# aiforvision/OCTA-autosegmentation

Hardware: AMD Instinct MI355X
Metric: synthetic OCTA samples/sec (graph + 304x304 image + 1216x1216 label triples) (higher is better)
Workload: dtype f64

## Files before the change

### include/octa_hip.h

```cpp
#ifndef OCTA_HIP_H
#define OCTA_HIP_H

#include <stddef.h>
#include <stdint.h>

#ifdef __cplusplus
extern "C" {
#endif

typedef struct octa_ctx octa_ctx;


int octa_abi_version(void);

const char *octa_last_error(void);

int octa_ctx_create(int device, octa_ctx **out);
void octa_ctx_destroy(octa_ctx *ctx);

size_t octa_ctx_scratch_bytes(const octa_ctx *ctx);

int octa_rasterize_2d(octa_ctx *ctx, int B, const double *d_edges, const int64_t *h_edge_off,
                      const uint8_t *d_keep, int no_pixels_x, int no_pixels_y, int mip_axis,
                      double min_radius, double max_radius, uint8_t *d_out, void *stream);
// ... 284 lines not shown
int octa_sim_geometry(int num_cus, int *h_out4);

int octa_sim_is_large(const octa_sim *sim);

int octa_sim_fields(octa_sim *sim, int sample, double *h_oxy, int64_t cap_oxy, int64_t *n_oxy, double *h_co2,
                    int64_t cap_co2, int64_t *n_co2);

int octa_sim_kat_kd_order(octa_ctx *ctx, const double *h_pts, int64_t n, const uint8_t *h_need, int32_t *h_indices);

int octa_sim_kat_kd_order_signflag(octa_ctx *ctx, const double *h_pts, int64_t n, const uint8_t *h_need, int32_t need_bits, int32_t *h_indices);

int octa_sim_kat_sample(octa_ctx *ctx, const double *h_cand, int64_t n_cand, const double *h_npos, const double *h_nrad, int64_t n_art,
                        double *h_oxy, int64_t n_oxy, int64_t cap_oxy, double eps_n, double eps_k, double eps_s, const double *h_cst8,
                        int64_t *h_n_out);

#ifdef __cplusplus
}
#endif
#endif
```

### octa_autosegmentation_amd/_native.py

```python
import contextlib
import ctypes
import os
import random as _random
import threading

import numpy as np

HERE = os.path.dirname(os.path.abspath(__file__))
LIB_PATH = os.environ.get("OCTA_HIP_LIB") or os.path.join(HERE, "liboctahip.so")

_lib = None
_ctxs = {}
_lock = threading.Lock()

c_void_p, c_int, c_double, c_size_t = ctypes.c_void_p, ctypes.c_int, ctypes.c_double, ctypes.c_size_t


def _struct(name, ints, ptrs):
    fields = [("struct_size", ctypes.c_uint32)] + [(k, c_int) for k in ints.split()] + [("slope", ctypes.c_float)] + [(k, c_void_p) for k in ptrs.split()]
    return type(name, (ctypes.Structure,), {"_fields_": fields})


Conv3x3Args = _struct("Conv3x3Args", "N H W Cin Cout stride in_dilation tap_mask out_scale out_off_y out_off_x C1 CY1 nslot",
                      "d_x d_x2 d_w d_y d_y2 d_scale1 d_shift1 d_scale2 d_shift2 d_stat_partials d_stat_slots d_residual")
# ... 113 lines not shown
    "octa_headn_nhwc_bwd": (c_int, [c_void_p, c_void_p, c_void_p, c_void_p, c_int, ctypes.c_int64, c_int, c_int, c_void_p, c_void_p, c_void_p, c_void_p]),
    "octa_conv3x3_c1_fwd": (c_int, [c_void_p, c_void_p, c_void_p, c_void_p, c_int, c_int, c_int, c_int, c_void_p, c_int, c_void_p]),
    "octa_fft2_c2c_f64_workspace_bytes": (c_size_t, [c_int, c_int, c_int]),
    "octa_fft2_c2c_f64": (c_int, [c_void_p, c_void_p, c_int, c_int, c_int, c_int, c_void_p, c_void_p]),
    "octa_oof_workspace_bytes": (c_size_t, [c_int, c_int, c_int]),
    "octa_oof_2d": (c_int, [c_void_p, c_void_p, c_int, c_int, c_int, c_void_p, c_void_p]),
    "octa_oof_2d_response": (c_int, [c_void_p, c_void_p, c_int, c_int, c_int, c_void_p, c_void_p]),
    "octa_frangi_workspace_bytes": (c_size_t, [c_int, c_int, c_int, c_int]),
    "octa_frangi_2d": (c_int, [c_void_p, c_void_p, c_int, c_int, c_int, c_int, c_void_p, c_void_p, ctypes.c_float, c_double, c_double, c_int, c_void_p, c_void_p]),
    "octa_frangi_hessian": (c_int, [c_void_p, c_void_p, c_void_p, c_void_p, c_int, c_int, c_int, c_int, c_void_p, ctypes.c_float, c_int, c_void_p, c_void_p]),
    "octa_frangi_eigenvalues": (c_int, [c_void_p, c_void_p, c_void_p, c_void_p, c_int, c_int, c_int, c_int, c_void_p, ctypes.c_float, c_int, c_void_p, c_void_p]),
    "octa_sim_kat_kd_order": (c_int, [c_void_p, c_void_p, ctypes.c_int64, c_void_p, c_void_p]),
    "octa_sim_kat_kd_order_signflag": (c_int, [c_void_p, c_void_p, ctypes.c_int64, c_void_p, ctypes.c_int32, c_void_p]),
    "octa_sim_kat_sample": (c_int, [c_void_p, c_void_p, ctypes.c_int64, c_void_p, c_void_p, ctypes.c_int64, c_void_p, ctypes.c_int64, ctypes.c_int64,
                                    c_double, c_double, c_double, c_void_p, c_void_p]),
}


class OctaHipError(RuntimeError):
    pass


def lib():
    global _lib
    if _lib is None:
        with _lock:
            if _lib is None:
                if not os.path.exists(LIB_PATH):
                    raise OctaHipError(
                        f"{LIB_PATH} is missing: build it with `python -m octa_autosegmentation_amd.build` "
# ... 113 lines not shown
```

### octa_autosegmentation_amd/csrc/sim.hip

```cpp

#include <chrono>
#include <vector>

#include "common.h"
#include "sim_host.h"
#include <thread>
#include <atomic>
#include <cstdlib>
#include <cstring>

using namespace OCTA_SIMK;

#if OCTA_SIM_LARGE
#define OCTA_SIM_T octa_simL_impl
#define OCTA_SIM_FN(name) octa_simL_##name
#else
#define OCTA_SIM_T octa_simS_impl
#define OCTA_SIM_FN(name) octa_simS_##name
#endif
#define octa_sim_create OCTA_SIM_FN(create)
#define octa_sim_destroy OCTA_SIM_FN(destroy)
#define octa_sim_run OCTA_SIM_FN(run)
#define octa_sim_run_states OCTA_SIM_FN(run_states)
#define octa_sim_np_state OCTA_SIM_FN(np_state)
#define octa_sim_edge_offsets OCTA_SIM_FN(edge_offsets)
#define octa_sim_export_edges OCTA_SIM_FN(export_edges)
#define octa_sim_export_edges_device OCTA_SIM_FN(export_edges_device)
#define octa_sim_trace OCTA_SIM_FN(trace)
#define octa_sim_stats OCTA_SIM_FN(stats)
#define octa_sim_kd_paths OCTA_SIM_FN(kd_paths)
#define octa_sim_assign_paths OCTA_SIM_FN(assign_paths)
#define octa_sim_fields OCTA_SIM_FN(fields)
#define octa_sim_service_stats OCTA_SIM_FN(service_stats)
#define octa_sim_geometry OCTA_SIM_FN(geometry)
#define octa_sim_spans OCTA_SIM_FN(spans)
#define octa_sim_timing OCTA_SIM_FN(timing)
#define octa_sim_kat_kd_order OCTA_SIM_FN(kat_kd_order)
#define octa_sim_kat_kd_order_signflag OCTA_SIM_FN(kat_kd_order_signflag)
#define octa_sim_kat_sample OCTA_SIM_FN(kat_sample)
struct OCTA_SIM_T;
extern "C" void octa_sim_destroy(OCTA_SIM_T *S);
extern "C" long long octa_sim_next_ticket(void);
extern "C" int *octa_sim_launch_flag(int device);

namespace {

constexpr int SIM_THREADS = SIM_THREADS_PER_WG;
constexpr int SIM_WG_PER_CU = 2;
#if OCTA_SIM_LARGE
constexpr size_t SIM_LDS = 2048;
#else
constexpr size_t SIM_LDS = SIM_LDS_BYTES;
static_assert((size_t)KD_MAILBOX_OFF + KD_MAILBOX_BYTES <= (size_t)SIM_USER_BYTES && SIM_WG_PER_CU * SIM_LDS <= 160 * 1024, "LDS budget");
#endif
// ... 1306 lines not shown
    hipLaunchKernelGGL(sim_kat_kd_kernel, dim3(1), dim3(SIM_THREADS), SIM_LDS, 0, d_pts, (int)n, d_need, d_idx, d_idx + n, d_xy, zlo, zhi, flag_in_sign, need_bits);
    OCTA_HIP_CHECK(hipGetLastError());
    std::vector<idx_t> h(n);
    OCTA_HIP_CHECK(hipMemcpy(h.data(), d_idx, sizeof(idx_t) * n, hipMemcpyDeviceToHost));
    for (int64_t i = 0; i < n; i++) h_indices[i] = (int32_t)h[i];
    (void)hipFree(d_pts); (void)hipFree(d_idx); (void)hipFree(d_xy); if (d_need) (void)hipFree(d_need);
    return 0;
}

__global__ void __launch_bounds__(SIM_THREADS)
sim_kat_sample_kernel(SimArrays A, SimConst C, IterParams P) {
    extern __shared__ __attribute__((aligned(16))) unsigned char smem[];
    Blk b = {(int)threadIdx.x, (int)blockDim.x, smem};
    phase_sample(b, A, C, P, 0);
}
}

extern "C" int octa_sim_kat_sample(octa_ctx *ctx, const double *h_cand, int64_t n_cand, const double *h_npos, const double *h_nrad, int64_t n_art,
                                   double *h_oxy, int64_t n_oxy, int64_t cap_oxy, double eps_n, double eps_k, double eps_s, const double *h_cst8,
                                   int64_t *h_n_out) {
    if (!ctx || !h_cst8 || !h_n_out || n_cand < 0 || n_cand > NCANDCAP || n_art < 0 || n_art > NCAP || n_oxy < 0 || n_oxy > OCAP || cap_oxy < n_oxy ||
        (n_cand && !h_cand) || (n_art && (!h_npos || !h_nrad)) || (cap_oxy && !h_oxy)) {
        octa::set_error("octa_sim_kat_sample: bad arguments");
        return -2;
    }
    OCTA_HIP_CHECK(hipSetDevice(ctx->device));
    SimConst C;
    memset(&C, 0, sizeof(C));
    C.ps = h_cst8[0]; C.sx = h_cst8[1]; C.sy = h_cst8[2]; C.sz = h_cst8[3]; C.gs = h_cst8[4]; C.fc0 = h_cst8[5]; C.fc1 = h_cst8[6];
    SampleScalars sc;
// ... 67 lines not shown
```

### octa_autosegmentation_amd/csrc/sim_api.cpp

```cpp
#include <cstdlib>
#include <cstring>
#include <new>

#include "common.h"

extern "C" {
struct octa_simS_impl;
struct octa_simL_impl;
#define OCTA_DECL(SFX, T)                                                                                                                       \
    int octa_sim##SFX##_create(octa_ctx *, const octa_sim_config *, int, T **);                                                                 \
    void octa_sim##SFX##_destroy(T *);                                                                                                          \
    int octa_sim##SFX##_run(T *, const uint32_t *, const uint64_t *, octa_bif_fn, void *, void *);                                              \
    int octa_sim##SFX##_run_states(T *, const double *, const double *, const uint32_t *, const uint32_t *, octa_bif_fn, void *, void *);       \
    int octa_sim##SFX##_np_state(T *, int, uint32_t *);                                                                                         \
    int octa_sim##SFX##_edge_offsets(T *, int64_t *, int64_t *);                                                                                \
    int octa_sim##SFX##_export_edges(T *, double *);                                                                                            \
    int octa_sim##SFX##_export_edges_device(T *, double *, void *);                                                                             \
    int octa_sim##SFX##_trace(T *, int32_t *);                                                                                                  \
    int octa_sim##SFX##_stats(T *, int64_t *);                                                                                                  \
    int octa_sim##SFX##_kd_paths(T *, int64_t *);                                                                                               \
    int octa_sim##SFX##_assign_paths(T *, int64_t *);                                                                                           \
    int octa_sim##SFX##_spans(T *, int64_t *);                                                                                                  \
    int octa_sim##SFX##_timing(T *, double *);                                                                                                  \
    int octa_sim##SFX##_service_stats(T *, double *);                                                                                           \
    int octa_sim##SFX##_geometry(int, int *);                                                                                                   \
    int octa_sim##SFX##_fields(T *, int, double *, int64_t, int64_t *, double *, int64_t, int64_t *);
OCTA_DECL(S, octa_simS_impl)
OCTA_DECL(L, octa_simL_impl)
#undef OCTA_DECL
int octa_simS_kat_kd_order(octa_ctx *, const double *, int64_t, const uint8_t *, int32_t *);
int octa_simS_kat_kd_order_signflag(octa_ctx *, const double *, int64_t, const uint8_t *, int32_t, int32_t *);
int octa_simS_kat_sample(octa_ctx *, const double *, int64_t, const double *, const double *, int64_t, double *, int64_t, int64_t, double, double, double,
                         const double *, int64_t *);
}

#include <atomic>
#include <mutex>
static std::atomic<long long> g_sim_launches{0};
extern "C" long long octa_sim_next_ticket(void) { return g_sim_launches.fetch_add(1, std::memory_order_acq_rel) + 1; }
extern "C" long long octa_sim_launch_count(void) { return g_sim_launches.load(std::memory_order_acquire); }
extern "C" int *octa_sim_launch_flag(int device) {
    static std::mutex m;
    static int *flags[64] = {};
    if (device < 0 || device >= 64) return nullptr;
    std::lock_guard<std::mutex> g(m);
    if (!flags[device]) {
        int prev = 0;
        if (hipGetDevice(&prev) != hipSuccess || hipSetDevice(device) != hipSuccess) return nullptr;
// ... 62 lines not shown
extern "C" int octa_sim_kd_paths(octa_sim *sim, int64_t *t) { NEED(sim, "octa_sim_kd_paths") return FWD(octa_simS_kd_paths(sim->s, t), octa_simL_kd_paths(sim->l, t)); }
extern "C" int octa_sim_assign_paths(octa_sim *sim, int64_t *t) { NEED(sim, "octa_sim_assign_paths") return FWD(octa_simS_assign_paths(sim->s, t), octa_simL_assign_paths(sim->l, t)); }
extern "C" int octa_sim_spans(octa_sim *sim, int64_t *t) { NEED(sim, "octa_sim_spans") return FWD(octa_simS_spans(sim->s, t), octa_simL_spans(sim->l, t)); }
extern "C" int octa_sim_timing(octa_sim *sim, double *t) { NEED(sim, "octa_sim_timing") return FWD(octa_simS_timing(sim->s, t), octa_simL_timing(sim->l, t)); }
extern "C" int octa_sim_service_stats(octa_sim *sim, double *t) { NEED(sim, "octa_sim_service_stats") return FWD(octa_simS_service_stats(sim->s, t), octa_simL_service_stats(sim->l, t)); }
extern "C" int octa_sim_fields(octa_sim *sim, int k, double *o, int64_t co, int64_t *no, double *c, int64_t cc, int64_t *nc) {
    NEED(sim, "octa_sim_fields") return FWD(octa_simS_fields(sim->s, k, o, co, no, c, cc, nc), octa_simL_fields(sim->l, k, o, co, no, c, cc, nc));
}
extern "C" int octa_sim_geometry(int num_cus, int *h_out4) { return octa_simS_geometry(num_cus, h_out4); }
extern "C" int octa_sim_kat_kd_order(octa_ctx *ctx, const double *p, int64_t n, const uint8_t *need, int32_t *o) { return octa_simS_kat_kd_order(ctx, p, n, need, o); }
extern "C" int octa_sim_kat_kd_order_signflag(octa_ctx *ctx, const double *p, int64_t n, const uint8_t *need, int32_t bits, int32_t *o) { return octa_simS_kat_kd_order_signflag(ctx, p, n, need, bits, o); }
extern "C" int octa_sim_kat_sample(octa_ctx *ctx, const double *cand, int64_t n_cand, const double *npos, const double *nrad, int64_t n_art, double *oxy,
                                   int64_t n_oxy, int64_t cap_oxy, double eps_n, double eps_k, double eps_s, const double *cst8, int64_t *n_out) {
    return octa_simS_kat_sample(ctx, cand, n_cand, npos, nrad, n_art, oxy, n_oxy, cap_oxy, eps_n, eps_k, eps_s, cst8, n_out);
}
extern "C" int octa_sim_is_large(const octa_sim *sim) { return sim && sim->large ? 1 : 0; }
```

### octa_autosegmentation_amd/csrc/sim_core.h

```cpp
#pragma once
#include <cmath>
#include <cstdint>
#include <cstring>
#include <algorithm>
#include "gpow.h"
#include "glibc_trig.h"

#ifndef OCTA_SIM_LARGE
#define OCTA_SIM_LARGE 0
#endif
#if OCTA_SIM_LARGE
#define OCTA_SIMK octa_simk_large
#else
#define OCTA_SIMK octa_simk
#endif
namespace OCTA_SIMK {

#if OCTA_SIM_LARGE
typedef unsigned int idx_t;
typedef unsigned long long kdw_t;
constexpr int IDX_BITS = 18;
constexpr int GROUP_BITS = 17;
constexpr int NCAP = 1 << 17;
constexpr int OCAP = 1 << 18;
// ... 282 lines not shown
    for (int i0 = s0; i0 < s1; i0 += 64) {
        const bool keep = i0 + lane < s1 && pred(i0 + lane);
        const unsigned long long m = __ballot(keep);
        if (keep) emit(i0 + lane, at + (int)__popcll(m & ((1ull << lane) - 1ull)));
        at += (int)__popcll(m);
    }
    return tot;
#else
    (void)b;
    int at = 0;
    for (int i = 0; i < n; i++) if (pred(i)) { emit(i, at); at++; }
    return at;
#endif
}

OCTA_HD inline void atomic_min_int(int *p, int v) {
#if defined(__HIP_DEVICE_COMPILE__)
    atomicMin(p, v);
#else
    if (v < *p) *p = v;
#endif
}
OCTA_HD inline int atomic_min_ret_int(int *p, int v) {
#if defined(__HIP_DEVICE_COMPILE__)
    return atomicMin(p, v);
#else
    int o = *p; if (v < o) *p = v; return o;
#endif
}
OCTA_HD inline int atomic_add_int(int *p, int v) {
// ... 661 lines not shown
#if defined(__HIP_DEVICE_COMPILE__)
    atomicMin(p, v);
#else
    if (v < *p) *p = v;
#endif
}

constexpr int KD_TAB_OFF = OCAP * (int)sizeof(kdw_t);
constexpr int KD_BOX_BYTES = KD_RANGES * 24;
static_assert(KD_RANGES >= OCAP / 17 + 1, "ranges per level");
static_assert(KD_MAILBOX_OFF % 16 == 0 && KD_MAILBOX_OFF >= KD_TAB_OFF + KD_RANGES * KD_TAB_BYTES_PER_RANGE, "kd tables overlap the mailbox");
static_assert(KD_MAILBOX_OFF + (KD_BOX_BYTES > KD_MAILBOX_BYTES ? KD_BOX_BYTES : KD_MAILBOX_BYTES) <= SIM_USER_BYTES, "kd table layout (box table and mailbox share their area)");
OCTA_HD inline void kd_build(const Blk &b, const double *pts, int n, idx_t *out_idx, idx_t *out_rank,
                              float *xy, double zlo, double zhi, long *kdprof = nullptr, const unsigned char *need = nullptr,
                              const bool flag_in_sign = false, const unsigned char need_bits = 0xff) {
#if defined(__HIP_DEVICE_COMPILE__) && !defined(OCTA_SIM_PROF_ASSIGN) && !defined(OCTA_SIM_PROF_SAMPLE) && !defined(OCTA_SIM_PROF_SET) && !defined(OCTA_SIM_PROF_MAIL) && !defined(OCTA_SIM_PROF_SEQ) && !defined(OCTA_SIM_PROF_SEQ2)
#define KDP(slot) do { if (kdprof && b.tid == 0) { long _t = (long)wall_clock64(); kdprof[slot] += _t - _kt; _kt = _t; } } while (0)
    long _kt = (long)wall_clock64();
#else
#define KDP(slot) do { } while (0)
#endif
    kdw_t *kv = reinterpret_cast<kdw_t *>(b.user_of<1>());
    idx_t *tab = reinterpret_cast<idx_t *>(b.user_of<1>() + KD_TAB_OFF);
    idx_t *rs = tab, *re = tab + KD_RANGES;
    idx_t *rs2 = tab + 2 * KD_RANGES, *re2 = tab + 3 * KD_RANGES;
    signed char *rd = reinterpret_cast<signed char *>(tab + 4 * KD_RANGES);
    unsigned *bbf = reinterpret_cast<unsigned *>(b.user_of<1>() + KD_MAILBOX_OFF);
#if defined(__HIP_DEVICE_COMPILE__) && !OCTA_SIM_LARGE
    if ((size_t)n * (sizeof(kdw_t) + 8) + 8 <= (size_t)KD_TAB_OFF)
        xy = reinterpret_cast<float *>(b.user_of<1>() + (((size_t)n * sizeof(kdw_t) + 7) & ~(size_t)7));
#endif
// ... 1717 lines not shown
                }
            }
            A.nn[a] = r;
            if (cached) {
                nn_prev[a] = r;
                if (r >= 0) nn_d2[a] = sqdist(ld3(G.src + 3 * r), p);
            }
        }
        b.sync();
        ASP(2);
    }
    int *fa = reinterpret_cast<int *>(b.user());
    static_assert((size_t)NCAP * 4 <= (size_t)SIM_USER_BYTES, "first-attractor table");
    for (int i = b.tid; i < n_nodes; i += b.nth) fa[i] = 0x7fffffff;
    b.sync();
    for (int a = b.tid; a < n_att; a += b.nth) { const int r = A.nn[a]; if (r >= 0) atomic_min_int(&fa[r], a); }
    b.sync();
    int n_groups = 0;
#if defined(__HIP_DEVICE_COMPILE__)
    {
        const int lane = b.tid & 63, wv = b.tid >> 6, nw = (b.nth + 63) >> 6;
        const int seg = ((n_att + nw * 64 - 1) / (nw * 64)) * 64;
        const int s0 = wv * seg < n_att ? wv * seg : n_att, s1 = s0 + seg < n_att ? s0 + seg : n_att;
        int cnt = 0;
        for (int a0 = s0; a0 < s1; a0 += 64) {
            const int a = a0 + lane;
            bool h = false;
            if (a < s1) { const int r = A.nn[a]; h = r >= 0 && fa[r] == a; }
            cnt += __popcll(__ballot(h));
        }
        int ex;
        n_groups = blk_scan(b, lane == 0 ? cnt : 0, &ex);
        int base = __builtin_amdgcn_readfirstlane(ex);
        for (int a0 = s0; a0 < s1; a0 += 64) {
            const int a = a0 + lane;
            bool h = false;
            int r = -1;
            if (a < s1) { r = A.nn[a]; h = r >= 0 && fa[r] == a; }
            const unsigned long long m = __ballot(h);
            if (h) {
                const int g = base + __popcll(m & ((1ull << lane) - 1ull));
                if (g < GCAP) { A.gnode[g] = r; fa[r] = -(g + 1); }
            }
            base += __popcll(m);
        }
    }
#else
    {
        const int chunk = (n_att + b.nth - 1) / b.nth;
        const int i0 = b.tid * chunk, i1 = (i0 + chunk < n_att) ? i0 + chunk : n_att;
        int local = 0;
        for (int a = i0; a < i1; a++) { int r = A.nn[a]; local += (r >= 0 && fa[r] == a) ? 1 : 0; }
        int ex;
        n_groups = blk_scan(b, local, &ex);
        int g = ex;
        for (int a = i0; a < i1; a++) {
            int r = A.nn[a];
            if (r >= 0 && fa[r] == a) {
                if (g < GCAP) { A.gnode[g] = r; fa[r] = -(g + 1); }
                g++;
            }
        }
    }
#endif
    b.sync();
    ASP(3);
    if (n_groups > GCAP) { if (b.tid == 0) atomic_or_int(&sc->err, ERR_GROUP_CAP); n_groups = GCAP; }
    int n_sorted = 0;
    auto book = [&](int *gc, int *cur, unsigned *srt, const bool staged) __attribute__((always_inline)) {
        for (int g = b.tid; g < n_groups; g += b.nth) gc[g] = 0;
        b.sync();
        for (int a = b.tid; a < n_att; a += b.nth) {
            const int r = A.nn[a];
            if (r >= 0) { const int v = fa[r]; if (v < 0) atomic_add_int(&gc[-v - 1], 1); }
        }
        b.sync();
        {
            const int chunk = ((n_groups + b.nth - 1) / b.nth) | 1;
            const int g0 = b.tid * chunk, g1 = (g0 + chunk < n_groups) ? g0 + chunk : n_groups;
            int local = 0;
            for (int g = g0; g < g1; g++) local += gc[g];
            int ex;
            n_sorted = blk_scan(b, local, &ex);
            int run = ex;
            for (int g = g0; g < g1; g++) { const int c = gc[g]; A.gstart[g] = run; cur[g] = run; if (staged) A.gcount[g] = c; run += c; }
        }
        b.sync();
        ASP(4);
        if (n_sorted > SORTCAP) { if (b.tid == 0) atomic_or_int(&sc->err, ERR_OXY_CAP); }
        for (int a = b.tid; a < n_att; a += b.nth) {
            const int r = A.nn[a];
            if (r >= 0) {
                const int v = fa[r];
                if (v < 0) { const int pos = atomic_add_int(&cur[-v - 1], 1); if (pos < SORTCAP) srt[pos] = (unsigned)a; }
            }
        }
        b.sync();
        ASP(5);
        for (int g = b.tid; g < n_groups; g += b.nth) {
            const int cnt = gc[g];
            unsigned *v = srt + (cur[g] - cnt);
            for (int i = 1; i < cnt; i++) {
                unsigned x = v[i];
                int j = i - 1;
                while (j >= 0 && v[j] > x) { v[j + 1] = v[j]; j--; }
                v[j + 1] = x;
            }
        }
        if (staged) {
            b.sync();
            const int n_out = n_sorted < SORTCAP ? n_sorted : SORTCAP;
// ... 229 lines not shown
    G.init_powers();
    const int ng = A.sc->n_groups[f];
    if (b.tid == 0) { A.sc->pass_counter++; A.sc->pass_tag[f] = A.sc->pass_counter; }
    b.sync();
    const int tag = A.sc->pass_tag[f];
    int n_grow = 0;
    idx_t *leaf = reinterpret_cast<idx_t *>(b.user());
    idx_t *posv = leaf + GCAP;
    unsigned char *keyv = reinterpret_cast<unsigned char *>(posv + GCAP);
    unsigned char *growf = keyv + GCAP;
    static_assert((size_t)2 * GCAP * sizeof(idx_t) + (size_t)2 * GCAP <= (size_t)SIM_USER_BYTES, "speculation lists");
    int *cnt = b.coll() + 110;
    static_assert(110 + 32 <= 396, "bucket counters in the collectives area");
    for (int k = b.tid; k < 32; k += b.nth) cnt[k] = 0;
    b.sync();
    for (int g = b.tid; g < ng; g += b.nth) {
        const int id = A.gnode[g];
        const int nch = A.nnch_of(f)[id], par = A.npar_of(f)[id];
        const int cls = nch == 0 ? 0 : ((par >= 0 && nch == 1) ? 1 : 2);
        int key = 32;
        if (cls == 2) {
            Rec R;
            memset(&R, 0, sizeof(R));
            R.type = 0; R.node = id; R.req = -1;
            A.rec[g] = R;
        } else {
            const int c = A.gcount[g];
            key = cls * 16 + (c < 15 ? c : 15);
            posv[g] = (idx_t)atomic_add_int(&cnt[key], 1);
        }
        keyv[g] = (unsigned char)key;
        growf[g] = 0;
    }
    b.sync();
    const int n_leaf = [&] { int t = 0; for (int k = 0; k < 16; k++) t += cnt[k]; return t; }();
    const int n_inter = [&] { int t = 0; for (int k = 16; k < 32; k++) t += cnt[k]; return t; }();
    b.sync();
    if (b.tid == 0) { int run = 0; for (int k = 0; k < 32; k++) { const int c = cnt[k]; cnt[k] = run; run += c; } }
    b.sync();
    for (int g = b.tid; g < ng; g += b.nth) {
        const int key = keyv[g];
        if (key < 32) leaf[cnt[key] + (int)posv[g]] = (idx_t)g;
    }
    b.sync();
    const idx_t *inter = leaf + n_leaf;
    for (int k = b.tid; k < n_leaf; k += b.nth) {
        const int g = (int)leaf[k];
// ... 355 lines not shown
        for (int i = b.tid; i < MURRAY_FLUSH_LDS / 32; i += b.nth) fl_done[i] = 0;
        b.sync();
        const int wv = b.tid >> 6;
        if (wv < 3 && wv * 64 < n) {
            const int rounds = murray_flush_rounds_wave(A.nrad_of(f), octa_gpow::LOG_TAB, octa_gpow::EXP_TAB, fl_val, fl_done, A.fl_rec + (size_t)f * MURRAY_FLUSH_LDS, n,
                                                        wv, 3, true);
            if (b.tid == 0) { A.sc->fl_pending[f] = 0; A.sc->flush_rounds += rounds; }
        }
        b.sync();
    }
#else
    (void)b; (void)A;
#endif
}

constexpr int COMPACT_TILE = 3072;
constexpr int COMPACT_TILE_NN = 2048;
OCTA_HD inline int compact_points(const Blk &b, double *pts, int n, const unsigned char *removed, double *stage, int *c_nn = nullptr,
                                  double *c_d2 = nullptr) {
    (void)stage;
    if (b.nth == 1) {
        int w = 0;
        for (int i = 0; i < n; i++)
            if (!removed[i]) {
                if (w != i) {
                    pts[3 * w] = pts[3 * i]; pts[3 * w + 1] = pts[3 * i + 1]; pts[3 * w + 2] = pts[3 * i + 2];
                    if (c_nn) { c_nn[w] = c_nn[i]; c_d2[w] = c_d2[i]; }
                }
                w++;
            }
        return w;
    }
    double *tile = reinterpret_cast<double *>(b.user_of<16>());
    static_assert((size_t)COMPACT_TILE * 24 <= (size_t)SIM_USER_BYTES && (size_t)COMPACT_TILE_NN * 36 <= (size_t)SIM_USER_BYTES, "compaction tile");
#if defined(__HIP_DEVICE_COMPILE__)
    const int lane = b.tid & 63, wv = b.tid >> 6, nw = (b.nth + 63) >> 6;
    const int TILE = c_nn ? COMPACT_TILE_NN : COMPACT_TILE;
    double *td = tile + 3 * COMPACT_TILE_NN;
    int *ti = reinterpret_cast<int *>(td + COMPACT_TILE_NN);
    int base = 0;
    for (int t0 = 0; t0 < n; t0 += TILE) {
        const int tn = n - t0 < TILE ? n - t0 : TILE;
        const int seg = ((tn + nw * 64 - 1) / (nw * 64)) * 64;
        const int s0 = t0 + (wv * seg < tn ? wv * seg : tn), s1 = s0 + seg < t0 + tn ? s0 + seg : t0 + tn;
        int c = 0;
        for (int i0 = s0; i0 < s1; i0 += 64) c += (int)__popcll(__ballot(i0 + lane < s1 && !removed[i0 + lane]));
        int ex;
        const int kept = blk_scan(b, lane == 0 ? c : 0, &ex);
        if (base != t0 || kept != tn) {
            int at = __builtin_amdgcn_readfirstlane(ex);
            constexpr int CB = 2;
            for (int i0 = s0; i0 < s1; i0 += CB * 64) {
                bool keep[CB];
                V3 v[CB];
                int vn[CB] = {};
                double vd[CB] = {};
#pragma unroll
                for (int u = 0; u < CB; u++) {
                    const int i = i0 + u * 64 + lane, ic = i < s1 ? i : s1 - 1;
                    keep[u] = i < s1 && !removed[ic];
                    v[u] = ld3(pts + 3 * (size_t)ic);
                    if (c_nn) { vn[u] = c_nn[ic]; vd[u] = c_d2[ic]; }
                }
// ... 4 lines not shown
                    if (keep[u]) {
                        const int w = at + (int)__popcll(m & ((1ull << lane) - 1ull));
                        tile[3 * w] = v[u].x; tile[3 * w + 1] = v[u].y; tile[3 * w + 2] = v[u].z;
                        if (c_nn) { ti[w] = vn[u]; td[w] = vd[u]; }
                    }
                    at += (int)__popcll(m);
                }
            }
            b.sync();
            for (int j = b.tid; j < kept * 3; j += b.nth) pts[(size_t)3 * base + j] = tile[j];
            if (c_nn)
                for (int j = b.tid; j < kept; j += b.nth) { c_nn[base + j] = ti[j]; c_d2[base + j] = td[j]; }
            b.sync();
        }
        base += kept;
    }
    return base;
#else
    (void)tile;
    return n;
#endif
}

OCTA_HD inline bool assign_memory_covers(const SimArrays &A, int f, int n) {
#ifdef OCTA_SIM_ASSIGN_NOCACHE
    (void)A; (void)f; (void)n;
    return false;
#else
    return OCTA_UNI((int)(A.nn_prev_of(f) != nullptr && A.sc->n_cached[f] == n)) != 0;
#endif
// ... 3 lines not shown
#define OCTA_SUBPROF(sc, slot, t0) do { if (b.tid == 0) { long _t1 = (long)wall_clock64(); (sc)->prof[slot] += _t1 - (t0); (t0) = _t1; } } while (0)
#define OCTA_SUBPROF_T0() ((long)wall_clock64())
#else
#define OCTA_SUBPROF(sc, slot, t0) do { (void)(t0); } while (0)
#define OCTA_SUBPROF_T0() 0L
#endif

OCTA_HD inline void phase_satisfy_art(const Blk &b, const SimArrays &A, const SimConst &C, const IterParams &P) {
    const double zext = C.sz;
    SampleScalars *sc = A.sc;
    const int nb = sc->new_begin[0], ne = sc->new_end[0];
    const int n_new = ne - nb, n_oxy = sc->n_oxy;
    if (n_new <= 0 || n_oxy <= 0) return;
    const double ek = P.eps_k, ek2 = ek * ek;
    long t0 = OCTA_SUBPROF_T0();
    for (int i = b.tid; i < n_oxy; i += b.nth) A.removed[i] = 0;
    int *ctl = b.coll() + 100;
    constexpr int HEAL_NONE = 0x7fffffff;
    if (b.tid == 0) { ctl[0] = 0; ctl[1] = 0; ctl[2] = 0; }
    unsigned char *xf = reinterpret_cast<unsigned char *>(A.nn);
    unsigned char *pf = xf + NCAP;
    static_assert((size_t)3 * NCAP <= (size_t)OCAP * sizeof(int), "group and pending flags fit the nearest-node list");
#ifdef OCTA_SIM_SET_NOHEAL
    constexpr bool HEAL = false;
#else
    constexpr bool HEAL = true;
#endif
    for (int j = b.tid; j < n_new && j < NCAP; j += b.nth) xf[j] = 0;
    b.sync();
    {
        int *new_ids = A.tmp_int;
        for (int j = b.tid; j < n_new; j += b.nth) new_ids[j] = nb + j;
        b.sync();
        Grid G = grid_build(b, A, A.npos[0], new_ids, n_new, ek);
        for (int o = b.tid; o < n_oxy; o += b.nth) {
            const V3 p = ld3(A.oxy + 3 * o);
            grid_visit(G, p.x, p.y, ek, [&](int j, const V3 &q) {
                if (sqdist(p, q) <= ek2) {
                    int slot = atomic_add_int(&ctl[0], 1);
                    if (slot < PCAP) A.pairs[slot] = ((unsigned)(j - nb) << IDX_BITS) | (unsigned)o;
                    A.removed[o] = 1;
                }
            });
        }
        b.sync();
    }
    OCTA_SUBPROF(sc, 12, t0);
    int n_pairs = ctl[0];
    if (n_pairs > PCAP) { if (b.tid == 0) atomic_or_int(&sc->err, ERR_PAIR_CAP); n_pairs = PCAP; }
    if (n_new > (1 << (32 - IDX_BITS))) { if (b.tid == 0) atomic_or_int(&sc->err, ERR_PAIR_CAP); }
    b.sync();
    if (n_pairs == 0) return;
    {
        const int n_ven = sc->n_nodes[1];
        int *rem = A.tmp_int;
        int n_rem = 0;
        {
            const int chunk = (n_oxy + b.nth - 1) / b.nth;
            const int i0 = b.tid * chunk < n_oxy ? b.tid * chunk : n_oxy, i1 = (i0 + chunk < n_oxy) ? i0 + chunk : n_oxy;
            int local = 0;
            for (int o = i0; o < i1; o++) local += A.removed[o] ? 1 : 0;
            int ex;
            n_rem = blk_scan(b, local, &ex);
            int run = ex;
            for (int o = i0; o < i1; o++) if (A.removed[o]) rem[run++] = o;
        }
        b.sync();
        for (int k = b.tid; k < n_rem; k += b.nth) {
            const int o = rem[k];
            A.ven_near[o] = 0;
            A.hashes[o] = py_hash_tuple3(ld3(A.oxy + 3 * o));
        }
        Grid G = grid_build(b, A, A.oxy, rem, n_rem, ek);
        constexpr int VB = 4;
        for (int j0 = b.tid; j0 < n_ven; j0 += VB * b.nth) {
            V3 qv[VB];
#pragma unroll
            for (int u = 0; u < VB; u++) { const int j = j0 + u * b.nth; qv[u] = ld3(A.npos[1] + 3 * (j < n_ven ? j : n_ven - 1)); }
#pragma unroll
            for (int u = 0; u < VB; u++) {
                if (j0 + u * b.nth >= n_ven) break;
                const V3 q = qv[u];
                grid_visit(G, q.x, q.y, ek, [&](int o, const V3 &p) {
                    if (sqrt(sqdist(q, p)) <= ek) A.ven_near[o] = 1;
                });
            }
        }
        b.sync();
    }
    OCTA_SUBPROF(sc, 12, t0);
    bool set_in_lds = false;
    int rung = 0;
    bool from_partial = false;
    auto sink_of = [&](unsigned pr) -> int {
        const unsigned low = pr & IDX_MASK;
        return (rung == 2 || (rung == 1 && xf[pr >> IDX_BITS])) ? (int)A.kd_idx[low] : (int)low;
    };
#ifdef OCTA_SIM_DEBUG_SAT
    int dbg_n_ins = -1, dbg_mask = -1, dbg_base = -1;
    const int dbg_n_co2_in = sc->n_co2;
#endif
    while (true) {
        const int vslot = rung == 1 ? 2 : 1;
// ... 390 lines not shown
            b.sync();
            loc = 0; for (int o = b.tid; o < n_oxy; o += b.nth) loc += mark[o];
            c_in_distinct = blk_scan(b, loc, &ex);
        }
        b.sync();
        if (b.tid == 0 && A.dbg) {
            int *row = A.dbg + 16 * A.dbg_it;
            row[0] = n_new; row[1] = n_oxy; row[2] = n_pairs; row[3] = c_rem; row[4] = c_ven; row[5] = c_pair_all; row[6] = c_pair_take;
            row[7] = c_pair_vs_removed; row[8] = dbg_n_ins; row[9] = dbg_mask; row[10] = dbg_base; row[11] = c_slots; row[12] = c_in_distinct;
            row[13] = c_slot_bad; row[14] = dbg_n_co2_in; row[15] = sc->n_co2;
        }
        b.sync();
    }
#endif
    const bool carry = assign_memory_covers(A, 0, n_oxy);
    int keep = compact_points(b, A.oxy, n_oxy, A.removed, A.tmp_dbl, carry ? A.nn_prev[0] : nullptr, carry ? A.nn_d2[0] : nullptr);
    if (b.tid == 0) { sc->n_oxy = keep; sc->n_cached[0] = carry ? keep : 0; }
    b.sync();
    OCTA_SUBPROF(sc, 15, t0);
}

OCTA_HD inline void phase_satisfy_ven(const Blk &b, const SimArrays &A, const IterParams &P) {
    SampleScalars *sc = A.sc;
    const int nb = sc->new_begin[1], ne = sc->new_end[1];
    const int n_new = ne - nb, n_co2 = sc->n_co2;
    if (n_new <= 0 || n_co2 <= 0) return;
    const double ek2 = P.eps_k * P.eps_k;
    const double ek = P.eps_k;
    {
        int *new_ids = A.tmp_int;
        for (int j = b.tid; j < n_new; j += b.nth) new_ids[j] = nb + j;
        b.sync();
        Grid G = grid_build(b, A, A.npos[1], new_ids, n_new, ek);
        for (int o = b.tid; o < n_co2; o += b.nth) {
            const V3 p = ld3(A.co2 + 3 * o);
            bool hit = false;
            grid_visit(G, p.x, p.y, ek, [&](int, const V3 &q) {
                if (!hit && sqdist(p, q) <= ek2) hit = true;
            });
            A.removed[o] = hit ? 1 : 0;
        }
        b.sync();
    }
    const bool carry = assign_memory_covers(A, 1, n_co2);
    int keep = compact_points(b, A.co2, n_co2, A.removed, A.tmp_dbl, carry ? A.nn_prev[1] : nullptr, carry ? A.nn_d2[1] : nullptr);
    if (b.tid == 0) { sc->n_co2 = keep; sc->n_cached[1] = carry ? keep : 0; }
    b.sync();
}

}
```

Baseline: 1657.

## Batch independent list loads per thread and build removed-oxygen list during the grid visit

Adds a `list_batch` helper that issues several independent global loads per thread before consuming them. It is applied to the attractor-grouping, booking, group-classification and oxygen-satisfy loops, to hide memory latency through more loads in flight. In the oxygen satisfy phase, the removed list, the ven_near reset and the hashes are now produced inside the grid visit via an atomic append. This replaces the separate clear pass, the block scan and the follow-up loop, but makes the order of the removed list nondeterministic. Also adds optional profiling macros and a self-test entry point for the batching helper.

```diff
diff --git a/include/octa_hip.h b/include/octa_hip.h
--- a/include/octa_hip.h
+++ b/include/octa_hip.h
@@ -322,6 +322,8 @@
                         double *h_oxy, int64_t n_oxy, int64_t cap_oxy, double eps_n, double eps_k, double eps_s, const double *h_cst8,
                         int64_t *h_n_out);
 
+int octa_sim_kat_list_batch(octa_ctx *ctx, int64_t n, int32_t *h_seen, int64_t *h_out3);
+
 #ifdef __cplusplus
 }
 #endif
diff --git a/octa_autosegmentation_amd/_native.py b/octa_autosegmentation_amd/_native.py
--- a/octa_autosegmentation_amd/_native.py
+++ b/octa_autosegmentation_amd/_native.py
@@ -151,6 +151,7 @@
     "octa_sim_kat_kd_order_signflag": (c_int, [c_void_p, c_void_p, ctypes.c_int64, c_void_p, ctypes.c_int32, c_void_p]),
     "octa_sim_kat_sample": (c_int, [c_void_p, c_void_p, ctypes.c_int64, c_void_p, c_void_p, ctypes.c_int64, c_void_p, ctypes.c_int64, ctypes.c_int64,
                                     c_double, c_double, c_double, c_void_p, c_void_p]),
+    "octa_sim_kat_list_batch": (c_int, [c_void_p, ctypes.c_int64, c_void_p, c_void_p]),
 }
 
 
diff --git a/octa_autosegmentation_amd/csrc/sim.hip b/octa_autosegmentation_amd/csrc/sim.hip
--- a/octa_autosegmentation_amd/csrc/sim.hip
+++ b/octa_autosegmentation_amd/csrc/sim.hip
@@ -38,6 +38,7 @@
 #define octa_sim_kat_kd_order OCTA_SIM_FN(kat_kd_order)
 #define octa_sim_kat_kd_order_signflag OCTA_SIM_FN(kat_kd_order_signflag)
 #define octa_sim_kat_sample OCTA_SIM_FN(kat_sample)
+#define octa_sim_kat_list_batch OCTA_SIM_FN(kat_list_batch)
 struct OCTA_SIM_T;
 extern "C" void octa_sim_destroy(OCTA_SIM_T *S);
 extern "C" long long octa_sim_next_ticket(void);
@@ -1374,6 +1375,38 @@
     Blk b = {(int)threadIdx.x, (int)blockDim.x, smem};
     phase_sample(b, A, C, P, 0);
 }
+
+__global__ void __launch_bounds__(SIM_THREADS)
+sim_kat_list_batch_kernel(const int *list, int n, int *seen, int *out) {
+    const int tid = (int)threadIdx.x, nth = (int)blockDim.x;
+    auto load = [&](int i) { atomicAdd(&out[1], 1); if (i < 0 || i >= n) { atomicAdd(&out[0], 1); return -1; } return list[i]; };
+    auto use = [&](int i, int v) { if (i < 0 || i >= n || v != 7 * i + 3) atomicAdd(&out[0], 1); else atomicAdd(&seen[i], 1); };
+    list_batch<LIST_AB, true>(tid, nth, n, load, use);
+    list_batch<LIST_AB, false>(tid, nth, n, load, use);
+}
+}
+
+extern "C" int octa_sim_kat_list_batch(octa_ctx *ctx, int64_t n, int32_t *h_seen, int64_t *h_out3) {
+    if (!ctx || !h_out3 || n < 0 || n > (1 << 20) || (n && !h_seen)) {
+        octa::set_error("octa_sim_kat_list_batch: bad arguments");
+        return -2;
+    }
+    OCTA_HIP_CHECK(hipSetDevice(ctx->device));
+    std::vector<int> h((size_t)n);
+    for (int64_t i = 0; i < n; i++) h[(size_t)i] = (int)(7 * i + 3);
+    int *d = nullptr;
+    OCTA_HIP_CHECK(hipMalloc(&d, sizeof(int) * (2 * (size_t)n + 2)));
+    int rc = 0;
+    auto ok = [&](hipError_t e, const char *what) { if (e != hipSuccess && rc == 0) { octa::set_error("octa_sim_kat_list_batch: %s: %s", what, hipGetErrorString(e)); rc = -1; } return rc == 0; };
+    int out[2] = {0, 0};
+    if (ok(hipMemset(d, 0, sizeof(int) * (2 * (size_t)n + 2)), "clear") && (!n || ok(hipMemcpy(d, h.data(), sizeof(int) * (size_t)n, hipMemcpyHostToDevice), "list"))) {
+        hipLaunchKernelGGL(sim_kat_list_batch_kernel, dim3(1), dim3(SIM_THREADS), 0, 0, d, (int)n, d + n, d + 2 * n);
+        if (ok(hipGetLastError(), "launch") && (!n || ok(hipMemcpy(h_seen, d + n, sizeof(int) * (size_t)n, hipMemcpyDeviceToHost), "visits")))
+            ok(hipMemcpy(out, d + 2 * n, sizeof(out), hipMemcpyDeviceToHost), "counts");
+    }
+    (void)hipFree(d);
+    h_out3[0] = out[0]; h_out3[1] = out[1]; h_out3[2] = LIST_AB;
+    return rc;
 }
 
 extern "C" int octa_sim_kat_sample(octa_ctx *ctx, const double *h_cand, int64_t n_cand, const double *h_npos, const double *h_nrad, int64_t n_art,
diff --git a/octa_autosegmentation_amd/csrc/sim_api.cpp b/octa_autosegmentation_amd/csrc/sim_api.cpp
--- a/octa_autosegmentation_amd/csrc/sim_api.cpp
+++ b/octa_autosegmentation_amd/csrc/sim_api.cpp
@@ -32,6 +32,7 @@
 int octa_simS_kat_kd_order_signflag(octa_ctx *, const double *, int64_t, const uint8_t *, int32_t, int32_t *);
 int octa_simS_kat_sample(octa_ctx *, const double *, int64_t, const double *, const double *, int64_t, double *, int64_t, int64_t, double, double, double,
                          const double *, int64_t *);
+int octa_simS_kat_list_batch(octa_ctx *, int64_t, int32_t *, int64_t *);
 }
 
 #include <atomic>
@@ -124,4 +125,5 @@
                                    int64_t n_oxy, int64_t cap_oxy, double eps_n, double eps_k, double eps_s, const double *cst8, int64_t *n_out) {
     return octa_simS_kat_sample(ctx, cand, n_cand, npos, nrad, n_art, oxy, n_oxy, cap_oxy, eps_n, eps_k, eps_s, cst8, n_out);
 }
+extern "C" int octa_sim_kat_list_batch(octa_ctx *ctx, int64_t n, int32_t *seen, int64_t *out3) { return octa_simS_kat_list_batch(ctx, n, seen, out3); }
 extern "C" int octa_sim_is_large(const octa_sim *sim) { return sim && sim->large ? 1 : 0; }
diff --git a/octa_autosegmentation_amd/csrc/sim_core.h b/octa_autosegmentation_amd/csrc/sim_core.h
--- a/octa_autosegmentation_amd/csrc/sim_core.h
+++ b/octa_autosegmentation_amd/csrc/sim_core.h
@@ -320,6 +320,36 @@
 #endif
 }
 
+#ifndef OCTA_SIM_LIST_BATCH
+#define OCTA_SIM_LIST_BATCH 8
+#endif
+constexpr int LIST_AB = OCTA_SIM_LIST_BATCH;
+static_assert(LIST_AB >= 1 && LIST_AB <= 16, "elements per thread and round");
+constexpr int LIST_AB_VISIT = LIST_AB < 4 ? LIST_AB : 4;
+template <int AB, bool UNROLL, class Load, class Use>
+OCTA_HD inline void list_batch(int tid, int nth, int n, Load &&load, Use &&use) {
+    for (int i0 = tid; i0 < n; i0 += AB * nth) {
+        decltype(load(0)) v[AB];
+#pragma unroll
+        for (int u = 0; u < AB; u++) { const int i = i0 + u * nth; v[u] = load(i < n ? i : n - 1); }
+        OCTA_ISSUE_LOADS();
+        if (UNROLL) {
+#pragma unroll
+            for (int u = 0; u < AB; u++) { const int i = i0 + u * nth; if (i < n) use(i, v[u]); }
+        } else {
+#pragma unroll 1
+            for (int u = 0; u < AB; u++) {
+                const int i = i0 + u * nth;
+                if (i >= n) break;
+                const decltype(load(0)) e = v[0];
+#pragma unroll
+                for (int k = 1; k < AB; k++) v[k - 1] = v[k];
+                use(i, e);
+            }
+        }
+    }
+}
+
 OCTA_HD inline void atomic_min_int(int *p, int v) {
 #if defined(__HIP_DEVICE_COMPILE__)
     atomicMin(p, v);
@@ -1011,7 +1041,7 @@
 OCTA_HD inline void kd_build(const Blk &b, const double *pts, int n, idx_t *out_idx, idx_t *out_rank,
                               float *xy, double zlo, double zhi, long *kdprof = nullptr, const unsigned char *need = nullptr,
                               const bool flag_in_sign = false, const unsigned char need_bits = 0xff) {
-#if defined(__HIP_DEVICE_COMPILE__) && !defined(OCTA_SIM_PROF_ASSIGN) && !defined(OCTA_SIM_PROF_SAMPLE) && !defined(OCTA_SIM_PROF_SET) && !defined(OCTA_SIM_PROF_MAIL) && !defined(OCTA_SIM_PROF_SEQ) && !defined(OCTA_SIM_PROF_SEQ2)
+#if defined(__HIP_DEVICE_COMPILE__) && !defined(OCTA_SIM_PROF_ASSIGN) && !defined(OCTA_SIM_PROF_SAMPLE) && !defined(OCTA_SIM_PROF_SET) && !defined(OCTA_SIM_PROF_MAIL) && !defined(OCTA_SIM_PROF_SEQ) && !defined(OCTA_SIM_PROF_SEQ2) && !defined(OCTA_SIM_PROF_SAT)
 #define KDP(slot) do { if (kdprof && b.tid == 0) { long _t = (long)wall_clock64(); kdprof[slot] += _t - _kt; _kt = _t; } } while (0)
     long _kt = (long)wall_clock64();
 #else
@@ -2759,7 +2789,7 @@
     static_assert((size_t)NCAP * 4 <= (size_t)SIM_USER_BYTES, "first-attractor table");
     for (int i = b.tid; i < n_nodes; i += b.nth) fa[i] = 0x7fffffff;
     b.sync();
-    for (int a = b.tid; a < n_att; a += b.nth) { const int r = A.nn[a]; if (r >= 0) atomic_min_int(&fa[r], a); }
+    list_batch<LIST_AB, true>(b.tid, b.nth, n_att, [&](int a) { return A.nn[a]; }, [&](int a, int r) { if (r >= 0) atomic_min_int(&fa[r], a); });
     b.sync();
     int n_groups = 0;
 #if defined(__HIP_DEVICE_COMPILE__)
@@ -2768,26 +2798,36 @@
         const int seg = ((n_att + nw * 64 - 1) / (nw * 64)) * 64;
         const int s0 = wv * seg < n_att ? wv * seg : n_att, s1 = s0 + seg < n_att ? s0 + seg : n_att;
         int cnt = 0;
-        for (int a0 = s0; a0 < s1; a0 += 64) {
-            const int a = a0 + lane;
-            bool h = false;
-            if (a < s1) { const int r = A.nn[a]; h = r >= 0 && fa[r] == a; }
-            cnt += __popcll(__ballot(h));
+        for (int a0 = s0; a0 < s1; a0 += LIST_AB * 64) {
+            int r[LIST_AB];
+#pragma unroll
+            for (int u = 0; u < LIST_AB; u++) { const int a = a0 + u * 64 + lane; r[u] = A.nn[a < s1 ? a : s1 - 1]; }
+            OCTA_ISSUE_LOADS();
+#pragma unroll
+            for (int u = 0; u < LIST_AB; u++) {
+                const int a = a0 + u * 64 + lane;
+                cnt += __popcll(__ballot(a < s1 && r[u] >= 0 && fa[r[u] >= 0 ? r[u] : 0] == a));
+            }
         }
         int ex;
         n_groups = blk_scan(b, lane == 0 ? cnt : 0, &ex);
         int base = __builtin_amdgcn_readfirstlane(ex);
-        for (int a0 = s0; a0 < s1; a0 += 64) {
-            const int a = a0 + lane;
-            bool h = false;
-            int r = -1;
-            if (a < s1) { r = A.nn[a]; h = r >= 0 && fa[r] == a; }
-            const unsigned long long m = __ballot(h);
-            if (h) {
-                const int g = base + __popcll(m & ((1ull << lane) - 1ull));
-                if (g < GCAP) { A.gnode[g] = r; fa[r] = -(g + 1); }
-            }
-            base += __popcll(m);
+        for (int a0 = s0; a0 < s1; a0 += LIST_AB * 64) {
+            int r[LIST_AB];
+#pragma unroll
+            for (int u = 0; u < LIST_AB; u++) { const int a = a0 + u * 64 + lane; r[u] = A.nn[a < s1 ? a : s1 - 1]; }
+            OCTA_ISSUE_LOADS();
+#pragma unroll
+            for (int u = 0; u < LIST_AB; u++) {
+                const int a = a0 + u * 64 + lane;
+                const bool h = a < s1 && r[u] >= 0 && fa[r[u] >= 0 ? r[u] : 0] == a;
+                const unsigned long long m = __ballot(h);
+                if (h) {
+                    const int g = base + __popcll(m & ((1ull << lane) - 1ull));
+                    if (g < GCAP) { A.gnode[g] = r[u]; fa[r[u]] = -(g + 1); }
+                }
+                base += __popcll(m);
+            }
         }
     }
 #else
@@ -2815,10 +2855,9 @@
     auto book = [&](int *gc, int *cur, unsigned *srt, const bool staged) __attribute__((always_inline)) {
         for (int g = b.tid; g < n_groups; g += b.nth) gc[g] = 0;
         b.sync();
-        for (int a = b.tid; a < n_att; a += b.nth) {
-            const int r = A.nn[a];
+        list_batch<LIST_AB, true>(b.tid, b.nth, n_att, [&](int a) { return A.nn[a]; }, [&](int, int r) {
             if (r >= 0) { const int v = fa[r]; if (v < 0) atomic_add_int(&gc[-v - 1], 1); }
-        }
+        });
         b.sync();
         {
             const int chunk = ((n_groups + b.nth - 1) / b.nth) | 1;
@@ -2833,13 +2872,12 @@
         b.sync();
         ASP(4);
         if (n_sorted > SORTCAP) { if (b.tid == 0) atomic_or_int(&sc->err, ERR_OXY_CAP); }
-        for (int a = b.tid; a < n_att; a += b.nth) {
-            const int r = A.nn[a];
+        list_batch<LIST_AB, true>(b.tid, b.nth, n_att, [&](int a) { return A.nn[a]; }, [&](int a, int r) {
             if (r >= 0) {
                 const int v = fa[r];
                 if (v < 0) { const int pos = atomic_add_int(&cur[-v - 1], 1); if (pos < SORTCAP) srt[pos] = (unsigned)a; }
             }
-        }
+        });
         b.sync();
         ASP(5);
         for (int g = b.tid; g < n_groups; g += b.nth) {
@@ -3099,23 +3137,37 @@
     static_assert(110 + 32 <= 396, "bucket counters in the collectives area");
     for (int k = b.tid; k < 32; k += b.nth) cnt[k] = 0;
     b.sync();
-    for (int g = b.tid; g < ng; g += b.nth) {
-        const int id = A.gnode[g];
-        const int nch = A.nnch_of(f)[id], par = A.npar_of(f)[id];
-        const int cls = nch == 0 ? 0 : ((par >= 0 && nch == 1) ? 1 : 2);
-        int key = 32;
-        if (cls == 2) {
-            Rec R;
-            memset(&R, 0, sizeof(R));
-            R.type = 0; R.node = id; R.req = -1;
-            A.rec[g] = R;
-        } else {
-            const int c = A.gcount[g];
-            key = cls * 16 + (c < 15 ? c : 15);
-            posv[g] = (idx_t)atomic_add_int(&cnt[key], 1);
-        }
-        keyv[g] = (unsigned char)key;
-        growf[g] = 0;
+    struct GroupKind { int id, c, nch, par; };
+    const unsigned char *nnch = A.nnch_of(f);
+    const int *npar = A.npar_of(f);
+    for (int g0 = b.tid; g0 < ng; g0 += LIST_AB * b.nth) {
+        GroupKind k[LIST_AB];
+#pragma unroll
+        for (int u = 0; u < LIST_AB; u++) { const int g = g0 + u * b.nth, gc = g < ng ? g : ng - 1; k[u].id = A.gnode[gc]; k[u].c = A.gcount[gc]; }
+        OCTA_ISSUE_LOADS();
+#pragma unroll
+        for (int u = 0; u < LIST_AB; u++) { k[u].nch = nnch[k[u].id]; k[u].par = npar[k[u].id]; }
+        OCTA_ISSUE_LOADS();
+#pragma unroll
+        for (int u = 0; u < LIST_AB; u++) {
+            const int g = g0 + u * b.nth;
+            if (g >= ng) break;
+            const int id = k[u].id, nch = k[u].nch, par = k[u].par;
+            const int cls = nch == 0 ? 0 : ((par >= 0 && nch == 1) ? 1 : 2);
+            int key = 32;
+            if (cls == 2) {
+                Rec R;
+                memset(&R, 0, sizeof(R));
+                R.type = 0; R.node = id; R.req = -1;
+                A.rec[g] = R;
+            } else {
+                const int c = k[u].c;
+                key = cls * 16 + (c < 15 ? c : 15);
+                posv[g] = (idx_t)atomic_add_int(&cnt[key], 1);
+            }
+            keyv[g] = (unsigned char)key;
+            growf[g] = 0;
+        }
     }
     b.sync();
     const int n_leaf = [&] { int t = 0; for (int k = 0; k < 16; k++) t += cnt[k]; return t; }();
@@ -3501,11 +3553,19 @@
 #endif
 }
 
+#if defined(OCTA_SIM_PROF_SAT) && defined(__HIP_DEVICE_COMPILE__)
+#define OCTA_SATP_T0() long _satp = (long)wall_clock64()
+#define OCTA_SATP(prof, set, slot) do { b.sync(); if (b.tid == 0) { long _t = (long)wall_clock64(); if ((OCTA_SIM_PROF_SAT + 0) == (set)) (prof)[slot] += _t - _satp; _satp = _t; } } while (0)
+#else
+#define OCTA_SATP_T0() do { } while (0)
+#define OCTA_SATP(prof, set, slot) do { } while (0)
+#endif
+
 constexpr int COMPACT_TILE = 3072;
 constexpr int COMPACT_TILE_NN = 2048;
 OCTA_HD inline int compact_points(const Blk &b, double *pts, int n, const unsigned char *removed, double *stage, int *c_nn = nullptr,
-                                  double *c_d2 = nullptr) {
-    (void)stage;
+                                  double *c_d2 = nullptr, long *satprof = nullptr) {
+    (void)stage; (void)satprof;
     if (b.nth == 1) {
         int w = 0;
         for (int i = 0; i < n; i++)
@@ -3526,6 +3586,7 @@
     double *td = tile + 3 * COMPACT_TILE_NN;
     int *ti = reinterpret_cast<int *>(td + COMPACT_TILE_NN);
     int base = 0;
+    OCTA_SATP_T0();
     for (int t0 = 0; t0 < n; t0 += TILE) {
         const int tn = n - t0 < TILE ? n - t0 : TILE;
         const int seg = ((tn + nw * 64 - 1) / (nw * 64)) * 64;
@@ -3534,6 +3595,7 @@
         for (int i0 = s0; i0 < s1; i0 += 64) c += (int)__popcll(__ballot(i0 + lane < s1 && !removed[i0 + lane]));
         int ex;
         const int kept = blk_scan(b, lane == 0 ? c : 0, &ex);
+        OCTA_SATP(satprof, 2, 0);
         if (base != t0 || kept != tn) {
             int at = __builtin_amdgcn_readfirstlane(ex);
             constexpr int CB = 2;
@@ -3568,6 +3630,7 @@
             b.sync();
         }
         base += kept;
+        OCTA_SATP(satprof, 2, 1);
     }
     return base;
 #else
@@ -3601,10 +3664,11 @@
     if (n_new <= 0 || n_oxy <= 0) return;
     const double ek = P.eps_k, ek2 = ek * ek;
     long t0 = OCTA_SUBPROF_T0();
-    for (int i = b.tid; i < n_oxy; i += b.nth) A.removed[i] = 0;
+    OCTA_SATP_T0();
     int *ctl = b.coll() + 100;
     constexpr int HEAL_NONE = 0x7fffffff;
-    if (b.tid == 0) { ctl[0] = 0; ctl[1] = 0; ctl[2] = 0; }
+    int *rem_n = b.coll() + 108;
+    if (b.tid == 0) { ctl[0] = 0; ctl[1] = 0; ctl[2] = 0; *rem_n = 0; }
     unsigned char *xf = reinterpret_cast<unsigned char *>(A.nn);
     unsigned char *pf = xf + NCAP;
     static_assert((size_t)3 * NCAP <= (size_t)OCAP * sizeof(int), "group and pending flags fit the nearest-node list");
@@ -3615,65 +3679,51 @@
 #endif
     for (int j = b.tid; j < n_new && j < NCAP; j += b.nth) xf[j] = 0;
     b.sync();
+    int *rem = A.tmp_int;
     {
         int *new_ids = A.tmp_int;
         for (int j = b.tid; j < n_new; j += b.nth) new_ids[j] = nb + j;
         b.sync();
+        OCTA_SATP(sc->kdprof, 1, 0);
         Grid G = grid_build(b, A, A.npos[0], new_ids, n_new, ek);
-        for (int o = b.tid; o < n_oxy; o += b.nth) {
-            const V3 p = ld3(A.oxy + 3 * o);
+        OCTA_SATP(sc->kdprof, 1, 1);
+        list_batch<LIST_AB_VISIT, false>(b.tid, b.nth, n_oxy, [&](int o) { return ld3(A.oxy + 3 * o); }, [&](int o, const V3 &p) {
+            bool hit = false;
             grid_visit(G, p.x, p.y, ek, [&](int j, const V3 &q) {
                 if (sqdist(p, q) <= ek2) {
                     int slot = atomic_add_int(&ctl[0], 1);
                     if (slot < PCAP) A.pairs[slot] = ((unsigned)(j - nb) << IDX_BITS) | (unsigned)o;
-                    A.removed[o] = 1;
+                    hit = true;
                 }
             });
-        }
+            A.removed[o] = hit ? 1 : 0;
+            if (hit) {
+                rem[atomic_add_int(rem_n, 1)] = o;
+                A.ven_near[o] = 0;
+                A.hashes[o] = py_hash_tuple3(p);
+            }
+        });
         b.sync();
+        OCTA_SATP(sc->kdprof, 1, 2);
     }
     OCTA_SUBPROF(sc, 12, t0);
     int n_pairs = ctl[0];
+    const int n_rem = OCTA_UNI(*rem_n);
     if (n_pairs > PCAP) { if (b.tid == 0) atomic_or_int(&sc->err, ERR_PAIR_CAP); n_pairs = PCAP; }
     if (n_new > (1 << (32 - IDX_BITS))) { if (b.tid == 0) atomic_or_int(&sc->err, ERR_PAIR_CAP); }
     b.sync();
     if (n_pairs == 0) return;
     {
         const int n_ven = sc->n_nodes[1];
-        int *rem = A.tmp_int;
-        int n_rem = 0;
-        {
-            const int chunk = (n_oxy + b.nth - 1) / b.nth;
-            const int i0 = b.tid * chunk < n_oxy ? b.tid * chunk : n_oxy, i1 = (i0 + chunk < n_oxy) ? i0 + chunk : n_oxy;
-            int local = 0;
-            for (int o = i0; o < i1; o++) local += A.removed[o] ? 1 : 0;
-            int ex;
-            n_rem = blk_scan(b, local, &ex);
-            int run = ex;
-            for (int o = i0; o < i1; o++) if (A.removed[o]) rem[run++] = o;
-        }
+        Grid G = grid_build(b, A, A.oxy, rem, n_rem, ek);
+        OCTA_SATP(sc->kdprof, 1, 5);
+        list_batch<LIST_AB_VISIT, false>(b.tid, b.nth, n_ven, [&](int j) { return ld3(A.npos[1] + 3 * j); }, [&](int, const V3 &q) {
+            grid_visit(G, q.x, q.y, ek, [&](int o, const V3 &p) {
+                if (sqrt(sqdist(q, p)) <= ek) A.ven_near[o] = 1;
+            });
+        });
         b.sync();
-        for (int k = b.tid; k < n_rem; k += b.nth) {
-            const int o = rem[k];
-            A.ven_near[o] = 0;
-            A.hashes[o] = py_hash_tuple3(ld3(A.oxy + 3 * o));
-        }
-        Grid G = grid_build(b, A, A.oxy, rem, n_rem, ek);
-        constexpr int VB = 4;
-        for (int j0 = b.tid; j0 < n_ven; j0 += VB * b.nth) {
-            V3 qv[VB];
-#pragma unroll
-            for (int u = 0; u < VB; u++) { const int j = j0 + u * b.nth; qv[u] = ld3(A.npos[1] + 3 * (j < n_ven ? j : n_ven - 1)); }
-#pragma unroll
-            for (int u = 0; u < VB; u++) {
-                if (j0 + u * b.nth >= n_ven) break;
-                const V3 q = qv[u];
-                grid_visit(G, q.x, q.y, ek, [&](int o, const V3 &p) {
-                    if (sqrt(sqdist(q, p)) <= ek) A.ven_near[o] = 1;
-                });
-            }
-        }
-        b.sync();
+        OCTA_SATP(sc->kdprof, 1, 6);
     }
     OCTA_SUBPROF(sc, 12, t0);
     bool set_in_lds = false;
@@ -4094,7 +4144,7 @@
     }
 #endif
     const bool carry = assign_memory_covers(A, 0, n_oxy);
-    int keep = compact_points(b, A.oxy, n_oxy, A.removed, A.tmp_dbl, carry ? A.nn_prev[0] : nullptr, carry ? A.nn_d2[0] : nullptr);
+    int keep = compact_points(b, A.oxy, n_oxy, A.removed, A.tmp_dbl, carry ? A.nn_prev[0] : nullptr, carry ? A.nn_d2[0] : nullptr, sc->kdprof);
     if (b.tid == 0) { sc->n_oxy = keep; sc->n_cached[0] = carry ? keep : 0; }
     b.sync();
     OCTA_SUBPROF(sc, 15, t0);
@@ -4111,7 +4161,9 @@
         int *new_ids = A.tmp_int;
         for (int j = b.tid; j < n_new; j += b.nth) new_ids[j] = nb + j;
         b.sync();
+        OCTA_SATP_T0();
         Grid G = grid_build(b, A, A.npos[1], new_ids, n_new, ek);
+        OCTA_SATP(sc->kdprof, 2, 2);
         for (int o = b.tid; o < n_co2; o += b.nth) {
             const V3 p = ld3(A.co2 + 3 * o);
             bool hit = false;
@@ -4121,9 +4173,10 @@
             A.removed[o] = hit ? 1 : 0;
         }
         b.sync();
+        OCTA_SATP(sc->kdprof, 2, 3);
     }
     const bool carry = assign_memory_covers(A, 1, n_co2);
-    int keep = compact_points(b, A.co2, n_co2, A.removed, A.tmp_dbl, carry ? A.nn_prev[1] : nullptr, carry ? A.nn_d2[1] : nullptr);
+    int keep = compact_points(b, A.co2, n_co2, A.removed, A.tmp_dbl, carry ? A.nn_prev[1] : nullptr, carry ? A.nn_d2[1] : nullptr, sc->kdprof);
     if (b.tid == 0) { sc->n_co2 = keep; sc->n_cached[1] = carry ? keep : 0; }
     b.sync();
 }
```

Result: no change. 1691 (median of 6 runs) (+2.1%).
